# elodin-sys/elodin

Hardware: AMD Instinct MI355X
Metric: entity-steps/s (6DOF RK4) (higher is better)
Workload: dtype f64

## Files before the change

### elodin_amd/csrc/kernels.hpp

```cpp
#pragma once
#include <hip/hip_runtime.h>
#include <stdint.h>

#pragma clang fp contract(on)

namespace sixdof {

constexpr int kMaxOps = 4;
constexpr int kMaxModelCols = 128;
constexpr int kBlock = 256;

struct DevOp {
    int32_t kind;
    int32_t aux_width;
    const void* aux;
    double p[6];
};

struct StepParams {
    void* pos;
    void* vel;
    void* accel;
    void* force;
    const void* inertia;
    uint32_t n;
    uint32_t n_ticks;
    double dt_g;
    double dt;
    uint32_t n_ops;
    uint32_t vel_independent;
    uint32_t streaming;
    uint32_t hist_ring;
    uint64_t hist_slot0;
    void* hist_pos;
    void* hist_vel;
    void* hist_accel;
    void* hist_force;
    uint64_t tick0;
    uint32_t accel_in_check;
    uint32_t reserved0;
    DevOp ops[kMaxOps];
    void* model_cols[kMaxModelCols];
    void* model_hist[kMaxModelCols];
};

enum : int { kRk4 = 0, kSemiImplicit = 1, kNone = 2 };

struct StepKernel {
    const void* fn = nullptr;
    dim3 grid;
};

StepKernel select_step(const StepParams& p, int integrator, int dtype);

hipError_t launch_step(const StepParams& p, int integrator, int dtype, hipStream_t stream);

using CustomAbiFn = unsigned (*)();
using CustomLayoutFn = unsigned (*)();
using CustomLaunchFn = int (*)(const StepParams*, int integrator, int dtype, void* stream);

constexpr int kPackWidth = 10;
constexpr int kPartialForce = 9;
constexpr int kPartialWidth = 18;

struct PairParams {
    void* pos;
    void* vel;
    void* accel;
    void* force;
    const void* inertia;
    uint32_t n;
    double dt_g, dt;
    double* pack;
    double* pack_next;
    double* partial;
    uint32_t splits;
    uint32_t partial_width;
    const uint32_t* row_start;
    const uint32_t* dst;
    uint32_t n_edges;
    uint32_t n_hubs, n_hub_chunks;
    const uint32_t* hub_rows;
    const uint32_t* hub_chunk_start;
    const uint32_t* chunk_e0;
    const uint32_t* chunk_row;
    double* chunk_partial;
    int32_t pair_kind;
    double p0, p1;
    uint32_t n_ops;
    DevOp ops[kMaxOps];
    uint32_t packed;
};
uint32_t pair_splits_for(uint32_t n);
// ... 38 lines not shown
```

### elodin_amd/csrc/sixdof_capi.cpp

```cpp
#include <dlfcn.h>
#include <hip/hip_runtime.h>

#include <algorithm>
#include <chrono>
#include <cmath>
#include <cstdio>
#include <cstdlib>
#include <cstring>
#include <iterator>
#include <map>
#include <string>
#include <unordered_map>
#include <vector>

#include "../../include/sixdof_hip.h"
#include "../../include/sixdof_apollo.h"
#include "kernels.hpp"
#include "abi_guard.hpp"
#include "aql_chain.hpp"
#include "step_plan.hpp"

using namespace sixdof;

namespace {

struct Column {
    uint64_t id = 0;
    int prim = SIXDOF_PRIM_F64;
    uint64_t width = 1;
    uint64_t n_rows = 0;
    size_t elem = 8;
    size_t bytes = 0;
    std::vector<uint64_t> ids;
    void* host = nullptr;
    void* dev = nullptr;
    std::vector<uint32_t> rows;
    uint32_t* d_rows = nullptr;
    void* compact = nullptr;
    void* live = nullptr;
    bool joined = false;
    void* snap = nullptr;
    bool host_pinned = false;
};

thread_local std::string g_create_error;

struct FoldTable {
    const uint32_t* src_rows;
    const uint32_t* row_start;
    const uint32_t* dst;
    uint32_t n_src;
    uint32_t n_lane;
};
constexpr uint32_t kFoldWaveDegree = 64;

struct FoldSlot {
    bool needs_table = false;
    bool wave_ok = false;
    uint32_t count = 1, stride = 0;
    bool set = false;
    uint32_t* d_blob = nullptr;
    FoldTable table{};
};
using SetFoldTableFn = int (*)(unsigned, const FoldTable*);

double now_ms() {
    using namespace std::chrono;
    return duration<double, std::milli>(steady_clock::now().time_since_epoch()).count();
}

uint64_t cid(const char* s) { return sixdof_component_id(s); }

constexpr uint32_t kAqlSlots = 8;

struct Replay {
    StepParams key{};
    std::map<uint32_t, hipGraphExec_t> graphs;
    bool aql_off = false;
    aql::Device* aql_dev = nullptr;
    std::string aql_why;
    std::string aql_fault;
    void* aql_args = nullptr;
    std::map<uint64_t, aql::Run> aql_runs;
    uint64_t aql_slot_key[kAqlSlots] = {};
    uint32_t aql_next_spare = 2;

    void drop() {
        for (auto& kv : graphs) hipGraphExecDestroy(kv.second);
        graphs.clear();
        aql_runs.clear();
        std::fill(std::begin(aql_slot_key), std::end(aql_slot_key), 0);
        aql_next_spare = 2;
    }
    void rekey(StepParams P) {
        P.tick0 = P.hist_slot0 = 0;
        if (std::memcmp(&P, &key, sizeof(P)) != 0) drop(), key = P;
    }
    void release() {
        drop();
        if (aql_args && aql_fault.empty()) hipFree(aql_args);
        aql::release(aql_dev);
    }
};

}

struct sixdof_handle {
    sixdof_desc desc{};
    int device = 0;
    hipStream_t stream = nullptr;
    hipEvent_t ev0 = nullptr, ev1 = nullptr;
    hipEvent_t evp0 = nullptr, evp1 = nullptr;
    bool prev_pending = false;
    hipStream_t copy_stream = nullptr;
    hipEvent_t ev_snap = nullptr, ev_copied = nullptr;
    bool copy_pending = false;
    uint64_t stream_lo = 0, stream_hi = 0;
    std::vector<void*> pinned_user;
    bool step_pending = false;
    std::vector<hipEvent_t> launch_events;
    std::map<uint64_t, Column> cols;
    std::vector<sixdof_effector_op> ops;
    std::vector<uint32_t> edge_src, edge_dst;
    std::vector<uint32_t> csr_start, csr_dst;
    uint32_t* d_csr_start = nullptr;
    uint32_t* d_csr_dst = nullptr;
    uint32_t* d_hub = nullptr;
    double* d_chunk_partial = nullptr;
    uint32_t n_hubs = 0, n_hub_chunks = 0;
    void* d_scratch = nullptr;
    size_t scratch_bytes = 0;
    std::vector<uint64_t> joined_ids;
    bool identity_join = true;
    uint64_t tick = 0;
    bool bound = false;
    bool resident = false;
    sixdof_timings last{};
    void* custom_dl = nullptr;
    CustomLaunchFn custom_launch = nullptr;
    void* pair_dl = nullptr;
    CustomPairLaunchFn pair_launch = nullptr;
    std::vector<uint64_t> custom_aux;
    std::vector<uint64_t> custom_model;
    bool custom_tick_free = false;
    int pair_only_small = -1;
// ... 97 lines not shown

uint32_t sixdof_abi_version(void) { return SIXDOF_ABI_VERSION; }


int sixdof_device_count(void) try {
    int n = 0;
    if (hipGetDeviceCount(&n) != hipSuccess) return 0;
    return n;
} SIXDOF_ABI_CATCH(&g_create_error)

const char* sixdof_last_error(const sixdof_handle* h) { return h ? h->err.c_str() : g_create_error.c_str(); }

void sixdof_destroy(sixdof_handle* h);

int sixdof_create(const sixdof_desc* d, sixdof_handle** out) try {
    if (!d || !out) {
        g_create_error = "sixdof_create: null argument";
        return SIXDOF_ERR_INVALID_ARGUMENT;
    }
    *out = nullptr;
    if (d->struct_size != sizeof(sixdof_desc)) {
        g_create_error = "sixdof_create: struct_size mismatch (ABI version skew)";
        return SIXDOF_ERR_INVALID_ARGUMENT;
    }
    if (d->integrator != SIXDOF_INTEGRATOR_RK4 && d->integrator != SIXDOF_INTEGRATOR_SEMI_IMPLICIT &&
        d->integrator != SIXDOF_INTEGRATOR_NONE) {
        g_create_error = "sixdof_create: unknown integrator";
        return SIXDOF_ERR_INVALID_ARGUMENT;
    }
    if (d->dtype != SIXDOF_F64 && d->dtype != SIXDOF_F32) {
        g_create_error = "sixdof_create: unknown dtype";
        return SIXDOF_ERR_INVALID_ARGUMENT;
    }
    if (d->n_entities > 0xFFFFFFF0ull) {
        g_create_error = "sixdof_create: n_entities exceeds u32 row index range";
        return SIXDOF_ERR_INVALID_ARGUMENT;
    }
    int n_dev = 0;
    hipError_t e = hipGetDeviceCount(&n_dev);
    if (e != hipSuccess || n_dev == 0) {
        g_create_error = std::string("sixdof_create: no HIP device (") + hipGetErrorString(e) +
                         "); this backend has no CPU fallback";
        return SIXDOF_ERR_NO_DEVICE;
    }
    if (d->device_ordinal < 0 || d->device_ordinal >= n_dev) {
        g_create_error = "sixdof_create: device_ordinal out of range";
        return SIXDOF_ERR_INVALID_ARGUMENT;
    }
    auto* h = new sixdof_handle();
    h->desc = *d;
    if (h->desc.ticks_per_launch == 0) h->desc.ticks_per_launch = 1;
    const char* aql_env = std::getenv("SIXDOF_AQL");
    h->replay.aql_off = aql_env && aql_env[0] == '0';
    h->device = d->device_ordinal;
    h->id_pos = cid("world_pos");
    h->id_vel = cid("world_vel");
    h->id_accel = cid("world_accel");
    h->id_force = cid("force");
    h->id_inertia = cid("inertia");
    h->id_tick = cid("tick");
    h->id_dt = cid("simulation_time_step");
    if ((e = hipSetDevice(h->device)) != hipSuccess || (e = hipStreamCreate(&h->stream)) != hipSuccess ||
        (e = hipEventCreate(&h->ev0)) != hipSuccess || (e = hipEventCreate(&h->ev1)) != hipSuccess ||
        (e = hipEventCreate(&h->evp0)) != hipSuccess || (e = hipEventCreate(&h->evp1)) != hipSuccess) {
        g_create_error = std::string("sixdof_create: ") + hipGetErrorString(e);
        sixdof_destroy(h);
        return SIXDOF_ERR_BACKEND;
    }
    *out = h;
    return SIXDOF_OK;
} SIXDOF_ABI_CATCH(&g_create_error)

void sixdof_destroy(sixdof_handle* h) try {
    if (!h) return;
    hipSetDevice(h->device);
    if (h->stream) hipStreamSynchronize(h->stream);
    h->replay.release();
    if (h->copy_stream) hipStreamSynchronize(h->copy_stream);
    for (auto& kv : h->cols) {
        h->free_join(kv.second);
        if (kv.second.dev) hipFree(kv.second.dev);
        if (kv.second.snap) hipFree(kv.second.snap);
        if (kv.second.host_pinned) hipHostUnregister(kv.second.host);
    }
    for (void* p : h->pinned_user) (void)hipHostUnregister(p);
    if (h->copy_stream) hipStreamDestroy(h->copy_stream);
    if (h->ev_snap) hipEventDestroy(h->ev_snap);
    if (h->ev_copied) hipEventDestroy(h->ev_copied);
    if (h->d_csr_start) hipFree(h->d_csr_start);
    if (h->d_csr_dst) hipFree(h->d_csr_dst);
    if (h->d_hub) hipFree(h->d_hub);
    if (h->d_chunk_partial) hipFree(h->d_chunk_partial);
    if (h->d_scratch) hipFree(h->d_scratch);
    if (h->d_tick_refs) hipFree(h->d_tick_refs);
    h->free_fold_tables();
    for (void* p : h->d_hist) if (p) hipFree(p);
    for (void* p : h->d_model_hist) if (p) hipFree(p);
    if (h->custom_dl) dlclose(h->custom_dl);
    if (h->pair_dl) dlclose(h->pair_dl);
    for (hipEvent_t e : h->launch_events) hipEventDestroy(e);
    if (h->ev0) hipEventDestroy(h->ev0);
    if (h->ev1) hipEventDestroy(h->ev1);
    if (h->evp0) hipEventDestroy(h->evp0);
    if (h->evp1) hipEventDestroy(h->evp1);
    if (h->stream) hipStreamDestroy(h->stream);
    delete h;
// ... 950 lines not shown
        const size_t slot0 = static_cast<size_t>((first_tick - 1) % h->hist_ring);
        const size_t head = std::min<size_t>(n_ticks, h->hist_ring - slot0);
        char* dst = static_cast<char*>(host_dst[k]);
        const char* ring = static_cast<const char*>(h->d_hist[k]);
        HIP_TRY(h, hipMemcpyAsync(dst, ring + slot0 * block, head * block, hipMemcpyDeviceToHost, h->copy_stream));
        if (head < n_ticks)
            HIP_TRY(h, hipMemcpyAsync(dst + head * block, ring, (n_ticks - head) * block, hipMemcpyDeviceToHost, h->copy_stream));
    }
    HIP_TRY(h, hipEventRecord(h->ev_copied, h->copy_stream));
    h->copy_pending = true;
    h->stream_lo = first_tick;
    h->stream_hi = last;
    return SIXDOF_OK;
} SIXDOF_ABI_CATCH(err_of(h))

int sixdof_download_column(sixdof_handle* h, uint64_t component_id) try {
    if (!h) return SIXDOF_ERR_INVALID_ARGUMENT;
    Column* c = h->col(component_id);
    if (!c) return h->fail(SIXDOF_ERR_COMPONENT_NOT_FOUND, "download_column: unknown component");
    HIP_TRY(h, hipSetDevice(h->device));
    int rc = scatter_back(h, c);
    if (rc != SIXDOF_OK) return rc;
    if (c->bytes) HIP_TRY(h, hipMemcpyAsync(c->host, c->dev, c->bytes, hipMemcpyDeviceToHost, h->stream));
    HIP_TRY(h, hipStreamSynchronize(h->stream));
    return SIXDOF_OK;
} SIXDOF_ABI_CATCH(err_of(h))

int sixdof_upload_column(sixdof_handle* h, uint64_t component_id) try {
    if (!h) return SIXDOF_ERR_INVALID_ARGUMENT;
    Column* c = h->col(component_id);
    if (!c) return h->fail(SIXDOF_ERR_COMPONENT_NOT_FOUND, "upload_column: unknown component");
    if (!h->resident) return h->fail(SIXDOF_ERR_INVALID_ARGUMENT, "upload_column: nothing is resident yet (sixdof_upload first)");
    HIP_TRY(h, hipSetDevice(h->device));
    if (c->bytes) HIP_TRY(h, hipMemcpyAsync(c->dev, c->host, c->bytes, hipMemcpyHostToDevice, h->stream));
    if (c->joined && c->compact) {
        hipError_t e = launch_gather_rows(c->compact, c->dev, c->d_rows, static_cast<uint32_t>(h->joined_ids.size()),
                                          static_cast<uint32_t>(c->width), c->elem, h->stream);
        if (e != hipSuccess) return h->hip_fail(e, "gather_rows");
    }
    HIP_TRY(h, hipStreamSynchronize(h->stream));
    if (component_id == h->id_accel) h->accel_is_host_data = true;
    return SIXDOF_OK;
} SIXDOF_ABI_CATCH(err_of(h))

bool graph_eligible(const sixdof_handle* h) {
    return (h->desc.flags & SIXDOF_FLAG_USE_GRAPH) && !(h->desc.flags & SIXDOF_FLAG_TIME_EACH_LAUNCH) && !h->hist_ring &&
           (h->custom_model.empty() || h->custom_tick_free) && h->model == 0 && !h->has_pair_op();
}

static bool opens_with_check(const sixdof_handle* h, uint64_t n_ticks) {
    return h->accel_is_host_data && h->desc.integrator == SIXDOF_INTEGRATOR_RK4 && n_ticks > 0;
}

constexpr size_t kGraphCacheMax = 8;

int ensure_graph(sixdof_handle* h, const StepParams& P, uint32_t len, hipGraphExec_t* out) {
    std::map<uint32_t, hipGraphExec_t>& graphs = h->replay.graphs;
    if (auto it = graphs.find(len); it != graphs.end()) {
        *out = it->second;
        return SIXDOF_OK;
    }
    if (graphs.size() >= kGraphCacheMax) {
        for (auto g = graphs.begin(); g != graphs.end();) {
            if (g->first == kGraphLen || g->first == kGraphLong) { ++g; continue; }
            hipGraphExecDestroy(g->second);
            g = graphs.erase(g);
        }
    }
    hipGraph_t g = nullptr;
    HIP_TRY(h, hipStreamBeginCapture(h->stream, hipStreamCaptureModeThreadLocal));
    hipError_t le = hipSuccess;
    for (uint32_t i = 0; i < len && le == hipSuccess; i++) le = launch_any(h, P);
    hipError_t ce = hipStreamEndCapture(h->stream, &g);
    if (le != hipSuccess) return h->hip_fail(le, "launch_step (capture)");
    if (ce != hipSuccess) return h->hip_fail(ce, "hipStreamEndCapture");
    hipGraphExec_t exec = nullptr;
    hipError_t ie = hipGraphInstantiate(&exec, g, nullptr, nullptr, 0);
    hipGraphDestroy(g);
    if (ie != hipSuccess) return h->hip_fail(ie, "hipGraphInstantiate");
    (void)hipGraphUpload(exec, h->stream);
    graphs[len] = exec;
    *out = exec;
    return SIXDOF_OK;
}

static int ensure_plan_graphs(sixdof_handle* h, const StepParams& P, const ChainPlan& c, hipGraphExec_t g[3]) {
    int rc = SIXDOF_OK;
    if (c.open || c.n_short) rc = ensure_graph(h, P, kGraphLen, &g[0]);
    if (rc == SIXDOF_OK && c.n_long) rc = ensure_graph(h, P, kGraphLong, &g[1]);
    if (rc == SIXDOF_OK && c.tail) rc = ensure_graph(h, P, c.tail, &g[2]);
    return rc;
}


constexpr size_t kAqlSlotBytes = (sizeof(StepParams) + 255) / 256 * 256;
constexpr double kAqlStallS = 60.0;

static bool aql_run(sixdof_handle* h, const StepParams& P, uint32_t check, uint32_t ticks, aql::Run* out) {
    Replay& rp = h->replay;
    const uint64_t key = uint64_t(check) << 32 | ticks;
    if (auto it = rp.aql_runs.find(key); it != rp.aql_runs.end()) return *out = it->second, true;
    uint32_t slot_index = check;
    if (ticks != h->desc.ticks_per_launch) {
        slot_index = rp.aql_next_spare;
        rp.aql_next_spare = slot_index + 1 == kAqlSlots ? 2 : slot_index + 1;
        rp.aql_runs.erase(rp.aql_slot_key[slot_index]);
        rp.aql_slot_key[slot_index] = 0;
    }
    StepParams Q = P;
    Q.accel_in_check = check;
    Q.n_ticks = ticks;
    Q.tick0 = Q.hist_slot0 = 0;
    const StepKernel k = select_step(Q, h->desc.integrator, h->desc.dtype);
    if (!k.fn) return rp.aql_why = "no built-in kernel for this launch", false;
    aql::Run r;
    if (!aql::kernel_code(rp.aql_dev, k.fn, sizeof(StepParams), &r.code, &rp.aql_why)) return false;
    if (r.code.kernarg_align > 256) return rp.aql_why = "kernarg alignment above 256 bytes", false;
    char* slot = static_cast<char*>(rp.aql_args) + slot_index * kAqlSlotBytes;
    hipError_t e = hipMemcpy(slot, &Q, sizeof(Q), hipMemcpyHostToDevice);
    if (e != hipSuccess) return rp.aql_why = std::string("hipMemcpy (argument block): ") + hipGetErrorString(e), false;
    r.kernarg = slot;
    r.blocks = k.grid.x;
    rp.aql_runs[key] = r;
    if (slot_index >= 2) rp.aql_slot_key[slot_index] = key;
    return *out = r, true;
}

static bool aql_batch(sixdof_handle* h, const StepParams& P, const BatchPlan& b, aql::Run runs[3]) {
    const uint32_t K = h->desc.ticks_per_launch;
    if ((b.check_ticks && !aql_run(h, P, 1, b.check_ticks, &runs[0])) || (b.full && !aql_run(h, P, 0, K, &runs[1])) ||
        (b.rem && !aql_run(h, P, 0, b.rem, &runs[2])))
        return false;
    runs[0].count = b.check_ticks ? 1 : 0;
    runs[1].count = b.full;
    runs[2].count = b.rem ? 1 : 0;
    return true;
}

enum class Path { kApollo, kPair, kAql, kRigid };

struct Route {
    Path path;
    const char* why = nullptr;
    int rc = SIXDOF_OK;
    BatchPlan plan{};
};

static Route choose_path(sixdof_handle* h, uint64_t n_ticks, StepParams* P, aql::Run runs[3]) {
    if (h->model == 1) return {Path::kApollo};
    if (h->has_pair_op()) return {Path::kPair};
    Replay& rp = h->replay;
    const bool replay = graph_eligible(h);
    const char* why = nullptr;
    if (rp.aql_off) why = "SIXDOF_AQL=0";
    else if (!replay) why = "not graph-eligible";
    else if (h->custom_launch) why = "generated pipe";
    else if (h->desc.flags & SIXDOF_FLAG_ASYNC_STEP) why = "ASYNC_STEP";
    else if (h->desc.n_entities == 0) why = "no rows";
    else if (!rp.aql_why.empty()) why = rp.aql_why.c_str();
    else if (!rp.aql_fault.empty()) return {Path::kAql};
    else if (!h->resident) why = "columns not uploaded yet";
    if (!h->bound) return {Path::kRigid, why, SIXDOF_ERR_COMPONENT_NOT_FOUND};
    if (int rc = fill_step_params(h, P); rc != SIXDOF_OK) return {Path::kRigid, why ? why : h->err.c_str(), rc};
    const uint32_t K = h->desc.ticks_per_launch;
    P->n_ticks = K;
    if (replay) rp.rekey(*P);
    const BatchPlan plan = plan_batch(n_ticks, K, opens_with_check(h, n_ticks), replay);
    if (!why && !rp.aql_dev && (rp.aql_dev = aql::acquire(h->device, &rp.aql_why))) {
        if (hipError_t e = hipMalloc(&rp.aql_args, kAqlSlots * kAqlSlotBytes); e != hipSuccess)
            rp.aql_args = nullptr, rp.aql_why = std::string("hipMalloc: ") + hipGetErrorString(e);
    }
    if (!why && (!rp.aql_why.empty() || !aql_batch(h, *P, plan, runs))) why = rp.aql_why.c_str();
    return {why ? Path::kRigid : Path::kAql, why, SIXDOF_OK, plan};
}

static int prepare_batch(sixdof_handle* h, const Route& r, const StepParams& P, uint64_t n_ticks) {
    if (r.path == Path::kAql && !h->replay.aql_fault.empty()) return SIXDOF_OK;
    aql::Run runs[3];
    hipGraphExec_t unused[3] = {};
    for (bool check : {false, opens_with_check(h, n_ticks)}) {
        const BatchPlan b = plan_batch(n_ticks, h->desc.ticks_per_launch, check, true);
        if (r.path == Path::kAql) (void)aql_batch(h, P, b, runs);
        else if (int rc = ensure_plan_graphs(h, P, b.chains, unused); rc != SIXDOF_OK) return rc;
    }
    if (r.path != Path::kAql) HIP_TRY(h, hipStreamSynchronize(h->stream));
    return SIXDOF_OK;
}

int prepare_graph(sixdof_handle* h) {
    if (!h->bound || !graph_eligible(h)) return SIXDOF_OK;
    StepParams P;
    aql::Run runs[3];
    const Route r = choose_path(h, h->desc.ticks_per_launch, &P, runs);
    if (r.rc != SIXDOF_OK) return SIXDOF_OK;
    if (r.path == Path::kAql) return prepare_batch(h, r, P, h->desc.ticks_per_launch);
    hipGraphExec_t unused = nullptr;
    int rc = ensure_graph(h, P, kGraphLen, &unused);
    if (rc == SIXDOF_OK) (void)hipStreamSynchronize(h->stream);
    return rc;
}

int sixdof_prepare_step(sixdof_handle* h, uint64_t n_ticks) try {
    if (!h) return SIXDOF_ERR_INVALID_ARGUMENT;
    if (!h->bound || !h->resident) return h->fail(SIXDOF_ERR_COMPONENT_NOT_FOUND, "prepare_step: upload the columns first");
    if (!graph_eligible(h)) return SIXDOF_OK;
    HIP_TRY(h, hipSetDevice(h->device));
    StepParams P;
    aql::Run runs[3];
    const Route r = choose_path(h, n_ticks, &P, runs);
    return r.rc != SIXDOF_OK ? r.rc : prepare_batch(h, r, P, n_ticks);
} SIXDOF_ABI_CATCH(err_of(h))

const char* sixdof_step_path(sixdof_handle* h) try {
    if (!h) return "invalid handle";
    (void)hipSetDevice(h->device);
    StepParams P;
    aql::Run runs[3];
    const Route r = choose_path(h, h->desc.ticks_per_launch, &P, runs);
    if (r.path == Path::kApollo) h->path = "apollo";
    else if (r.path == Path::kPair) h->path = "pair";
    else if (r.path == Path::kAql) h->path = h->replay.aql_fault.empty() ? "aql" : "aql (failed: " + h->replay.aql_fault + ")";
    else h->path = std::string(graph_eligible(h) ? "hipgraph: " : "eager: ") + r.why;
    return h->path.c_str();
} SIXDOF_ABI_CATCH_VALUE(err_of(h), nullptr)

static int step_pair(sixdof_handle* h, uint64_t n_ticks, uint64_t* launches) {
    if (h->desc.dtype != SIXDOF_F64) return h->fail(SIXDOF_ERR_UNSUPPORTED, "step: pair effectors are f64 only");
    PairParams P;
    int rc = fill_pair_params(h, &P);
    if (rc != SIXDOF_OK) return rc;
    const char* no_small = std::getenv("SIXDOF_PAIR_SMALL");
    const bool custom = P.pair_kind == SIXDOF_EFF_EDGE_CUSTOM;
    bool small = P.n <= kPairSmallMax && !(no_small && no_small[0] == '0');
    if (custom) {
        if (!h->pair_launch) return h->fail(SIXDOF_ERR_BACKEND, "step: custom pair op without sixdof_set_custom_pair");
        if (h->pair_only_small >= 0) small = h->pair_only_small == 1;
        if (small && P.n > kPairSmallMax)
            return h->fail(SIXDOF_ERR_INVALID_ARGUMENT, "step: the pair object was generated for the one-launch small-graph kernel (<= " +
                           std::to_string(kPairSmallMax) + " rows) but the joined graph has " + std::to_string(P.n) + " rows");
    }
    const uint32_t K = h->hist_ring ? 1u : (small ? h->desc.ticks_per_launch : 1u << 20);
    const bool sets_packed = custom || !small;
    for (uint64_t done = 0; done < n_ticks;) {
        const uint32_t k = static_cast<uint32_t>(std::min<uint64_t>(K, n_ticks - done));
        if (custom) {
            hipError_t e = static_cast<hipError_t>(h->pair_launch(&P, h->desc.integrator, k, small ? 1 : 0, h->stream, launches));
            if (e != hipSuccess) return h->hip_fail(e, "custom pair launch");
        } else if (small) {
            hipError_t e = launch_pair_small(P, h->desc.integrator, k, h->stream, launches);
            if (e != hipSuccess) return h->hip_fail(e, "launch_pair_small");
        } else {
            hipError_t e = launch_pair_ticks(P, h->desc.integrator, k, h->stream, launches);
            if (e != hipSuccess) return h->hip_fail(e, "launch_pair_ticks");
        }
        done += k;
        if (sets_packed) P.packed = 1;
        if (int src = snapshot_tick_to_ring(h, h->tick + done); src != SIXDOF_OK) return src;
    }
    return SIXDOF_OK;
}

static int step_rigid(sixdof_handle* h, const StepParams& P, const BatchPlan& b, uint64_t n_ticks, uint64_t* launches) {
    const uint32_t K = h->desc.ticks_per_launch;
    const bool time_each = (h->desc.flags & SIXDOF_FLAG_TIME_EACH_LAUNCH) != 0;
    if (time_each) {
        const uint64_t need = 2 * b.launches();
        if (need > 8192) return h->fail(SIXDOF_ERR_INVALID_ARGUMENT, "step: TIME_EACH_LAUNCH supports <= 4096 launches per call");
        while (h->launch_events.size() < need) {
            hipEvent_t e = nullptr;
            HIP_TRY(h, hipEventCreate(&e));
            h->launch_events.push_back(e);
        }
    }
    auto eager = [&](StepParams Q, uint32_t ticks) -> int {
        Q.n_ticks = ticks;
        Q.tick0 = Q.hist_slot0 = h->tick + *launches * K;
        if (time_each) HIP_TRY(h, hipEventRecord(h->launch_events[2 * *launches], h->stream));
        hipError_t e = launch_any(h, Q);
        if (e != hipSuccess) return h->hip_fail(e, "launch_step");
        if (time_each) HIP_TRY(h, hipEventRecord(h->launch_events[2 * *launches + 1], h->stream));
        ++*launches;
        return SIXDOF_OK;
    };
    if (n_ticks > 0) h->accel_is_host_data = false;
    if (b.check_ticks) {
        StepParams P1 = P;
        P1.accel_in_check = 1;
        if (int rc = eager(P1, b.check_ticks); rc != SIXDOF_OK) return rc;
    }
    if (const ChainPlan& c = b.chains; c.launches()) {
        hipGraphExec_t g[3] = {};
        if (int rc = ensure_plan_graphs(h, P, c, g); rc != SIXDOF_OK) return rc;
        HIP_TRY(h, hipEventRecord(h->ev0, h->stream));
        const std::pair<hipGraphExec_t, uint64_t> replays[4] = {{g[0], c.open ? 1 : 0}, {g[1], c.n_long}, {g[0], c.n_short}, {g[2], c.tail ? 1 : 0}};
        for (const auto& [graph, times] : replays)
            for (uint64_t i = 0; i < times; i++) HIP_TRY(h, hipGraphLaunch(graph, h->stream));
        *launches += c.launches();
    }
    h->last.graph_launches = b.chains.launches();
    for (uint64_t i = b.chains.launches(); i < b.full; i++)
        if (int rc = eager(P, K); rc != SIXDOF_OK) return rc;
    return b.rem ? eager(P, b.rem) : SIXDOF_OK;
}

static int step_aql(sixdof_handle* h, const BatchPlan& b, const aql::Run runs[3], uint64_t n_ticks, uint64_t* launches) {
    Replay& rp = h->replay;
    if (!rp.aql_fault.empty()) return h->fail(SIXDOF_ERR_BACKEND, rp.aql_fault);
    for (hipStream_t s : {h->stream, static_cast<hipStream_t>(nullptr)}) {
        const hipError_t q = hipStreamQuery(s);
        if (q == hipErrorNotReady) HIP_TRY(h, hipStreamSynchronize(s));
        else if (q != hipSuccess) return h->hip_fail(q, "hipStreamQuery");
    }
    double device_ms = 0.0;
    if (!aql::run_chain(rp.aql_dev, runs, 3, kAqlStallS, &device_ms, &rp.aql_fault))
        return h->fail(SIXDOF_ERR_BACKEND, rp.aql_fault);
    if (n_ticks > 0) h->accel_is_host_data = false;
    *launches = b.launches();
    h->last.graph_launches = b.chains.launches();
    h->last.kernel_device_ms = device_ms;
    return SIXDOF_OK;
}

int sixdof_step(sixdof_handle* h, uint64_t n_ticks, sixdof_timings* tm) try {
    if (!h) return SIXDOF_ERR_INVALID_ARGUMENT;
    if (!h->bound) return h->fail(SIXDOF_ERR_COMPONENT_NOT_FOUND, "step: no columns bound");
    HIP_TRY(h, hipSetDevice(h->device));
    const double t0 = now_ms();
    const bool async_step = (h->desc.flags & SIXDOF_FLAG_ASYNC_STEP) != 0;
    if (h->step_pending || h->prev_pending) {
        std::swap(h->ev0, h->evp0);
        std::swap(h->ev1, h->evp1);
        std::swap(h->step_pending, h->prev_pending);
        if (h->step_pending) {
            float ms_prev = 0.f;
            HIP_TRY(h, hipEventSynchronize(h->ev1));
            if (hipEventElapsedTime(&ms_prev, h->ev0, h->ev1) == hipSuccess) h->last.kernel_device_ms = ms_prev;
            h->step_pending = false;
        }
    }
    if (h->hist_ring && h->copy_pending && h->stream_hi >= h->stream_lo && n_ticks) {
        const uint64_t ring = h->hist_ring, in_flight = h->stream_hi - h->stream_lo + 1;
        const uint64_t a = h->tick % ring, b = (h->stream_lo - 1) % ring;
        const uint64_t gap_ab = (b + ring - a) % ring, gap_ba = (a + ring - b) % ring;
        const bool overlap = n_ticks + in_flight > ring || gap_ab < std::min<uint64_t>(n_ticks, ring) || gap_ba < in_flight;
        if (overlap) HIP_TRY(h, hipStreamWaitEvent(h->stream, h->ev_copied, 0));
    }
    if (h->desc.integrator == SIXDOF_INTEGRATOR_NONE && (!h->custom_launch || h->model != 0 || h->has_pair_op()))
        return h->fail(SIXDOF_ERR_UNSUPPORTED, "step: SIXDOF_INTEGRATOR_NONE runs generated system programs only (sixdof_set_custom_pipe)");
    uint64_t launches = 0;
    StepParams P;
    aql::Run runs[3];
    const Route r = choose_path(h, n_ticks, &P, runs);
    if (r.rc != SIXDOF_OK) return r.rc;
    const bool aql = r.path == Path::kAql;
    if (!aql) HIP_TRY(h, hipEventRecord(h->ev0, h->stream));
    const int rc = aql                       ? step_aql(h, r.plan, runs, n_ticks, &launches)
                   : r.path == Path::kApollo ? step_apollo(h, n_ticks, &launches)
                   : r.path == Path::kPair   ? step_pair(h, n_ticks, &launches)
                                             : step_rigid(h, P, r.plan, n_ticks, &launches);
    if (rc != SIXDOF_OK) return rc;
    if (!aql) HIP_TRY(h, hipEventRecord(h->ev1, h->stream));
    if (!async_step && !aql) {
        const double spin_until = now_ms() + 0.25;
        hipError_t q = hipEventQuery(h->ev1);
        while (q == hipErrorNotReady && now_ms() < spin_until) q = hipEventQuery(h->ev1);
        if (q != hipSuccess) {
            (void)hipGetLastError();
            HIP_TRY(h, hipStreamSynchronize(h->stream));
        }
        float ms0 = 0.f;
        hipEventElapsedTime(&ms0, h->ev0, h->ev1);
        h->last.kernel_device_ms = ms0;
    }
    h->tick += n_ticks;
    h->step_pending = async_step;
    h->last.kernel_invoke_ms = now_ms() - t0;
    h->last.launches = launches;
    h->last.ticks = n_ticks;
    h->last.kernel_sum_ms = 0.0;
    if ((h->desc.flags & SIXDOF_FLAG_TIME_EACH_LAUNCH) && !h->has_pair_op()) {
        for (uint64_t i = 0; i < launches && 2 * i + 1 < h->launch_events.size(); i++) {
            float one = 0.f;
            if (hipEventElapsedTime(&one, h->launch_events[2 * i], h->launch_events[2 * i + 1]) == hipSuccess) h->last.kernel_sum_ms += one;
        }
    }
    if (tm) *tm = h->last;
    return SIXDOF_OK;
} SIXDOF_ABI_CATCH(err_of(h))


static thread_local sixdof_handle* g_tick_handle = nullptr;

int sixdof_tick_bind(sixdof_handle* h) try {
    g_tick_handle = h;
    return SIXDOF_OK;
} SIXDOF_ABI_CATCH(err_of(h))

static void tick_slot_ids(const sixdof_handle* h, std::vector<uint64_t>* in, std::vector<uint64_t>* out) {
    *in = {h->id_tick, h->id_force, h->id_inertia, h->id_pos, h->id_dt, h->id_vel, h->id_accel};
    for (auto& o : h->ops)
        if (o.aux_component_id) in->push_back(o.aux_component_id);
    std::map<uint64_t, int> ordered;
    for (uint64_t id : *in) ordered[id] = 1;
    out->clear();
// ... 59 lines not shown
```

### elodin_amd/csrc/step_kernel.hpp

```cpp
#pragma once
#include <type_traits>

#include "effectors.hpp"
#include "kernels.hpp"
#include "spatial.hpp"

namespace sixdof {

constexpr int kWave = 64;

typedef __attribute__((address_space(1))) const void* global_cptr;
typedef __attribute__((address_space(3))) void* lds_ptr;


constexpr int kPolPlain = 0, kPolNtStores = 1, kPolSc1Stores = 2, kPolNt = 9;
constexpr int pol_ld(int pol) { return pol / 8; }
constexpr int pol_st(int pol) { return pol % 8; }

template <int BYTES, int POL>
__device__ __forceinline__ void slab_dma_in(const char* __restrict__ g, char* l, uint32_t lane) {
    constexpr int kFull = BYTES / 1024, kRem = (BYTES % 1024) / 16;
    constexpr int kAux = pol_ld(POL) == 1 ? 2 : 0;
#pragma unroll
    for (int i = 0; i < kFull; i++)
// ... 108 lines not shown
    Quat<T> q0 = {T(0), T(0), T(0), T(1)};
    Vec3<T> p0 = {T(0), T(0), T(0)}, inv_I = {T(1), T(1), T(1)}, I_diag = {T(1), T(1), T(1)};
    Spatial<T> v0 = zero6, A_out = zero6, F_out = zero6;
    T mass = T(1), inv_m = T(1);
    if (active && !kDead) {
        const T* r = l_pos + t * 7;
        q0 = Quat<T>{r[0], r[1], r[2], r[3]};
        p0 = Vec3<T>{r[4], r[5], r[6]};
        const T* s = l_vel + t * 6;
        v0.ang = Vec3<T>{s[0], s[1], s[2]};
        v0.lin = Vec3<T>{s[3], s[4], s[5]};
        const T* m = l_c + t * 7;
        I_diag = Vec3<T>{m[0], m[1], m[2]};
        inv_I = Vec3<T>{recip(m[0]), recip(m[1]), recip(m[2])};
        mass = m[6];
        inv_m = recip(mass);
        if constexpr (INTEGRATOR == kNone || PIPE::kPreReadsAccel) {
            const T* a = g_accel + (size_t)t * 6;
            A_out = Spatial<T>{{a[0], a[1], a[2]}, {a[3], a[4], a[5]}};
        }
        if constexpr (INTEGRATOR == kNone) {
            const T* f = g_force + (size_t)t * 6;
            F_out = Spatial<T>{{f[0], f[1], f[2]}, {f[3], f[4], f[5]}};
        }
    }
    if (P.n_ticks == 0) return;
    __syncthreads();

    auto stage_pos = [&](const Quat<T>& q, const Vec3<T>& p) {
        if (active) {
            T* r = l_pos + t * 7;
            r[0] = q.i; r[1] = q.j; r[2] = q.k; r[3] = q.w; r[4] = p.x; r[5] = p.y; r[6] = p.z;
        }
    };
    auto stage6 = [&](T* l, const Spatial<T>& m) {
        if (active) {
            T* s = l + t * 6;
            s[0] = m.ang.x; s[1] = m.ang.y; s[2] = m.ang.z; s[3] = m.lin.x; s[4] = m.lin.y; s[5] = m.lin.z;
        }
    };
    auto flush7 = [&](const T* l, T* o, auto pol) {
        if (full) slab_out<ROWS * 7 * sizeof(T), decltype(pol)::value>(reinterpret_cast<const char*>(l), reinterpret_cast<char*>(o), t);
        else slab_out_tail(l, o, rows * 7, t);
    };
    auto flush6 = [&](const T* l, T* o, auto pol) {
        if (full) slab_out<ROWS * 6 * sizeof(T), decltype(pol)::value>(reinterpret_cast<const char*>(l), reinterpret_cast<char*>(o), t);
        else slab_out_tail(l, o, rows * 6, t);
    };
    constexpr std::integral_constant<int, POL> kLive{};
    constexpr std::integral_constant<int, 1> kRing{};

    const bool record = P.hist_pos != nullptr && P.hist_ring != 0;
    const bool early_ok = !PIPE::kHasModel && !record && !(P.streaming & 256u);
    const T dt_g = T(P.dt_g), dt = T(P.dt);
    Body<T> b;
    b.mass = mass;
    b.I = I_diag;
    Wrench<T> F = zero_wrench<T>();
    bool flushed = false;
#ifdef SIXDOF_TICK_OUT_OF_LINE
    auto one_tick = [&](auto early_tag, auto check_tag, uint32_t tick) __attribute__((noinline)) {
#else
    auto one_tick = [&](auto early_tag, auto check_tag, uint32_t tick) {
#endif
        constexpr bool early = decltype(early_tag)::value;
        const bool check = decltype(check_tag)::value || (PIPE::kHasModel && P.accel_in_check && tick == 0);
        if constexpr (PIPE::kHasModel) {
            PIPE::pre(P, P.tick0 + tick + 1, regs, q0, p0, v0, I_diag, mass, A_out);
            if constexpr (PIPE::kWritesInertia) {
                inv_I = Vec3<T>{recip(I_diag.x), recip(I_diag.y), recip(I_diag.z)};
                inv_m = recip(mass);
                b.mass = mass;
                b.I = I_diag;
            }
        }
        if constexpr (INTEGRATOR == kRk4) {
            const T h1 = dt_g * T(0.5), h3 = dt_g;
            Spatial<T> A, sv, sa;
            b.q = normalized(q0);
            b.p = p0;
            b.v = v0;
            if (check && active) {
                const T* a = g_accel + (size_t)t * 6;
                b.v.ang = b.v.ang + T(0) * Vec3<T>{a[0], a[1], a[2]};
                b.v.lin = b.v.lin + T(0) * Vec3<T>{a[3], a[4], a[5]};
            }
            F = zero_wrench<T>();
            PIPE::apply(P, aux, regs, b, F);
            A = calc_accel<PIPE>(b.q, F, inv_I, inv_m, T(0));
            sv = b.v;
            sa = A;
            b.q = integrate_world(q0, h1 * v0.ang);
            b.p = axpy(h1, v0.lin, p0);
            b.v = axpy(h1, A, v0);
            sv = axpy(T(2), b.v, sv);
            F = zero_wrench<T>();
            PIPE::apply(P, aux, regs, b, F);
            A = calc_accel<PIPE>(b.q, F, inv_I, inv_m, T(0));
            sa = axpy(T(2), A, sa);
            b.v = axpy(h1, A, v0);
            sv = axpy(T(2), b.v, sv);
            if (!PIPE::vel_independent(P)) {
                F = zero_wrench<T>();
                PIPE::apply(P, aux, regs, b, F);
                A = calc_accel<PIPE>(b.q, F, inv_I, inv_m, T(0));
            }
            sa = axpy(T(2), A, sa);
            T n3;
            b.q = integrate_world(q0, h3 * v0.ang, &n3);
            const T taint = accel_taint(n3);
            b.p = axpy(h3, v0.lin, p0);
            b.v = axpy(h3, A, v0);
            sv = sv + b.v;
            const T g = dt * T(1.0 / 6.0);
            const Quat<T> q_new = integrate_world(q0, g * sv.ang);
            const Vec3<T> p_new = axpy(g + taint, sv.lin, p0);
            if constexpr (early) {
                stage_pos(q_new, p_new);
                __syncthreads();
                flush7(l_pos, g_pos, kLive);
            }
            F = zero_wrench<T>();
            PIPE::apply(P, aux, regs, b, F);
            if constexpr (early) {
                stage6(l_force, world_wrench<PIPE>(b.q, F));
                __syncthreads();
                flush6(l_force, g_force, kLive);
            }
            A = calc_accel<PIPE>(b.q, F, inv_I, inv_m + taint, taint);
            if constexpr (early) {
                stage6(l_c, A);
                __syncthreads();
                flush6(l_c, g_accel, kLive);
            }
            sa = sa + A;
            v0 = axpy(g, sa, v0);
            q0 = q_new;
            p0 = p_new;
            A_out = A;
            if constexpr (early) {
                stage6(l_vel, v0);
                __syncthreads();
                flush6(l_vel, g_vel, kLive);
                flushed = true;
            }
        } else if constexpr (INTEGRATOR == kNone) {
        } else {
            T n0;
            b.q = normalized(q0, &n0);
            const T taint = accel_taint(n0);
            b.p = p0;
            b.v = v0;
            F = zero_wrench<T>();
            PIPE::apply(P, aux, regs, b, F);
            if constexpr (early) {
                stage6(l_force, world_wrench<PIPE>(b.q, F));
                __syncthreads();
                flush6(l_force, g_force, kLive);
            }
            const Spatial<T> A = calc_accel<PIPE>(b.q, F, inv_I, inv_m + taint, taint);
            if constexpr (early) {
                stage6(l_c, A);
                __syncthreads();
                flush6(l_c, g_accel, kLive);
            }
            v0 = axpy(dt, A, v0);
            if constexpr (early) {
                stage6(l_vel, v0);
                __syncthreads();
                flush6(l_vel, g_vel, kLive);
            }
            q0 = integrate_world(q0, dt * v0.ang);
            p0 = axpy(dt, v0.lin, p0);
            A_out = A;
            if constexpr (early) {
                stage_pos(q0, p0);
                __syncthreads();
                flush7(l_pos, g_pos, kLive);
                flushed = true;
            }
        }
        if constexpr (PIPE::kHasModel) PIPE::post(P, P.tick0 + tick + 1, regs, q0, p0, v0, I_diag, mass, A_out);
        if (record) {
            if constexpr (INTEGRATOR != kNone) F_out = world_wrench<PIPE>(b.q, F);
            const size_t slot = (size_t)((P.hist_slot0 + tick) % P.hist_ring);
            if constexpr (!kDead) {
                stage_pos(q0, p0);
                stage6(l_vel, v0);
                stage6(l_c, A_out);
                stage6(l_force, F_out);
                __syncthreads();
                const size_t r7 = (slot * P.n + row0) * 7, r6 = (slot * P.n + row0) * 6;
                flush7(l_pos, static_cast<T*>(P.hist_pos) + r7, kRing);
                flush6(l_vel, static_cast<T*>(P.hist_vel) + r6, kRing);
                flush6(l_c, static_cast<T*>(P.hist_accel) + r6, kRing);
                flush6(l_force, static_cast<T*>(P.hist_force) + r6, kRing);
            }
            if constexpr (PIPE::kHasModel)
                if (active) PIPE::record(P, slot, row0 + t, regs);
            __syncthreads();
        }
    };
    {
        constexpr std::false_type no{};
        constexpr std::true_type yes{};
        uint32_t tick = 0;
        if constexpr (PIPE::kHasModel) {
            for (; tick < P.n_ticks; tick++) one_tick(no, no, tick);
        } else {
            if constexpr (INTEGRATOR == kRk4 && CHECK)
                if (P.accel_in_check && P.n_ticks) one_tick(no, yes, tick++);
            for (; tick + 1 < P.n_ticks; tick++) one_tick(no, no, tick);
            if (tick < P.n_ticks) {
                if (early_ok) one_tick(yes, no, tick);
                else one_tick(no, no, tick);
            }
        }
    }
    if constexpr (PIPE::kHasModel) {
        if (active) {
            PIPE::template store<T, POL>(P, row0 + t, regs);
            if constexpr (PIPE::kWritesInertia) {
                T* gi = static_cast<T*>(const_cast<void*>(P.inertia)) + (size_t)(row0 + t) * 7;
                gi[0] = I_diag.x; gi[1] = I_diag.y; gi[2] = I_diag.z; gi[6] = mass;
            }
        }
    }
    if (flushed || kDead) return;
    if constexpr (INTEGRATOR != kNone) F_out = world_wrench<PIPE>(b.q, F);
    stage_pos(q0, p0);
    stage6(l_vel, v0);
    stage6(l_c, A_out);
    stage6(l_force, F_out);
    __syncthreads();
    flush7(l_pos, g_pos, kLive);
    flush6(l_vel, g_vel, kLive);
    flush6(l_c, g_accel, kLive);
    flush6(l_force, g_force, kLive);
}


template <class T, class PIPE, int POL>
inline StepKernel select_i(const StepParams& p, int integrator, dim3 grid) {
#ifdef SIXDOF_AB_BUILD
    if constexpr (!PIPE::kHasModel) {
        if ((p.streaming & 512u) && integrator == kRk4 && !p.accel_in_check)
            return {reinterpret_cast<const void*>(&sixdof_step_kernel<T, kRk4, PIPE, POL, false, 32>), dim3((p.n + 31) / 32)};
    }
#endif
    if (integrator == kRk4) {
        if constexpr (!PIPE::kHasModel) {
            if (p.accel_in_check)
                return {reinterpret_cast<const void*>(&sixdof_step_kernel<T, kRk4, PIPE, kPolPlain, true>), grid};
        }
        return {reinterpret_cast<const void*>(&sixdof_step_kernel<T, kRk4, PIPE, POL>), grid};
    }
    if (integrator == kNone) {
        if constexpr (PIPE::kHasModel) return {reinterpret_cast<const void*>(&sixdof_step_kernel<T, kNone, PIPE, POL>), grid};
        return {};
    }
    return {reinterpret_cast<const void*>(&sixdof_step_kernel<T, kSemiImplicit, PIPE, POL>), grid};
}

template <class T, class PIPE, bool SWEEP>
inline StepKernel select_t(const StepParams& p, int integrator, dim3 grid) {
    const uint32_t pol = p.streaming & 255u;
    switch (pol) {
    case kPolNt: return select_i<T, PIPE, kPolNt>(p, integrator, grid);
    case kPolNtStores: return select_i<T, PIPE, kPolNtStores>(p, integrator, grid);
    default: break;
    }
#ifdef SIXDOF_AB_BUILD
    if (pol == kPolSc1Stores) return select_i<T, PIPE, kPolSc1Stores>(p, integrator, grid);
    if constexpr (SWEEP) {
        switch (pol) {
        case 3: return select_i<T, PIPE, 3>(p, integrator, grid);
        case 4: return select_i<T, PIPE, 4>(p, integrator, grid);
        case 8: return select_i<T, PIPE, 8>(p, integrator, grid);
        case 10: return select_i<T, PIPE, 10>(p, integrator, grid);
        case 11: return select_i<T, PIPE, 11>(p, integrator, grid);
        case 12: return select_i<T, PIPE, 12>(p, integrator, grid);
        default: break;
        }
    }
#endif
    return select_i<T, PIPE, kPolPlain>(p, integrator, grid);
}

template <class PIPE, bool SWEEP = false>
// ... 7 lines not shown
```

Baseline: 13.26 billion.

## Skip accel and force writes on non-final launches in multi-launch batches

```diff
diff --git a/elodin_amd/csrc/kernels.hpp b/elodin_amd/csrc/kernels.hpp
--- a/elodin_amd/csrc/kernels.hpp
+++ b/elodin_amd/csrc/kernels.hpp
@@ -38,7 +38,7 @@
     void* hist_force;
     uint64_t tick0;
     uint32_t accel_in_check;
-    uint32_t reserved0;
+    uint32_t state_only;
     DevOp ops[kMaxOps];
     void* model_cols[kMaxModelCols];
     void* model_hist[kMaxModelCols];
diff --git a/elodin_amd/csrc/sixdof_capi.cpp b/elodin_amd/csrc/sixdof_capi.cpp
--- a/elodin_amd/csrc/sixdof_capi.cpp
+++ b/elodin_amd/csrc/sixdof_capi.cpp
@@ -72,10 +72,12 @@
 uint64_t cid(const char* s) { return sixdof_component_id(s); }
 
 constexpr uint32_t kAqlSlots = 8;
+constexpr uint32_t kAqlSpare0 = 3;
 
 struct Replay {
     StepParams key{};
     std::map<uint32_t, hipGraphExec_t> graphs;
+    bool state_only_off = false;
     bool aql_off = false;
     aql::Device* aql_dev = nullptr;
     std::string aql_why;
@@ -83,14 +85,14 @@
     void* aql_args = nullptr;
     std::map<uint64_t, aql::Run> aql_runs;
     uint64_t aql_slot_key[kAqlSlots] = {};
-    uint32_t aql_next_spare = 2;
+    uint32_t aql_next_spare = kAqlSpare0;
 
     void drop() {
         for (auto& kv : graphs) hipGraphExecDestroy(kv.second);
         graphs.clear();
         aql_runs.clear();
         std::fill(std::begin(aql_slot_key), std::end(aql_slot_key), 0);
-        aql_next_spare = 2;
+        aql_next_spare = kAqlSpare0;
     }
     void rekey(StepParams P) {
         P.tick0 = P.hist_slot0 = 0;
@@ -294,6 +296,8 @@
     if (h->desc.ticks_per_launch == 0) h->desc.ticks_per_launch = 1;
     const char* aql_env = std::getenv("SIXDOF_AQL");
     h->replay.aql_off = aql_env && aql_env[0] == '0';
+    const char* so_env = std::getenv("SIXDOF_STATE_ONLY");
+    h->replay.state_only_off = so_env && so_env[0] == '0';
     h->device = d->device_ordinal;
     h->id_pos = cid("world_pos");
     h->id_vel = cid("world_vel");
@@ -1350,25 +1354,37 @@
     return h->accel_is_host_data && h->desc.integrator == SIXDOF_INTEGRATOR_RK4 && n_ticks > 0;
 }
 
+static bool state_only_eligible(const sixdof_handle* h) {
+    return !h->replay.state_only_off && !h->custom_launch && !h->hist_ring && h->model == 0 && !h->has_pair_op();
+}
+
 constexpr size_t kGraphCacheMax = 8;
 
-int ensure_graph(sixdof_handle* h, const StepParams& P, uint32_t len, hipGraphExec_t* out) {
+enum class Chain : uint32_t { kAll = 0, kStateOnly = 1, kClosing = 2 };
+static uint32_t graph_key(uint32_t len, Chain v) { return len << 2 | static_cast<uint32_t>(v); }
+
+int ensure_graph(sixdof_handle* h, const StepParams& P, uint32_t len, Chain variant, hipGraphExec_t* out) {
     std::map<uint32_t, hipGraphExec_t>& graphs = h->replay.graphs;
-    if (auto it = graphs.find(len); it != graphs.end()) {
+    if (auto it = graphs.find(graph_key(len, variant)); it != graphs.end()) {
         *out = it->second;
         return SIXDOF_OK;
     }
     if (graphs.size() >= kGraphCacheMax) {
         for (auto g = graphs.begin(); g != graphs.end();) {
-            if (g->first == kGraphLen || g->first == kGraphLong) { ++g; continue; }
+            if (g->first >> 2 == kGraphLen || g->first >> 2 == kGraphLong) { ++g; continue; }
             hipGraphExecDestroy(g->second);
             g = graphs.erase(g);
         }
     }
+    StepParams Q = P;
+    Q.state_only = variant == Chain::kAll ? 0u : 1u;
     hipGraph_t g = nullptr;
     HIP_TRY(h, hipStreamBeginCapture(h->stream, hipStreamCaptureModeThreadLocal));
     hipError_t le = hipSuccess;
-    for (uint32_t i = 0; i < len && le == hipSuccess; i++) le = launch_any(h, P);
+    for (uint32_t i = 0; i < len && le == hipSuccess; i++) {
+        if (i + 1 == len && variant == Chain::kClosing) Q.state_only = 0;
+        le = launch_any(h, Q);
+    }
     hipError_t ce = hipStreamEndCapture(h->stream, &g);
     if (le != hipSuccess) return h->hip_fail(le, "launch_step (capture)");
     if (ce != hipSuccess) return h->hip_fail(ce, "hipStreamEndCapture");
@@ -1377,36 +1393,58 @@
     hipGraphDestroy(g);
     if (ie != hipSuccess) return h->hip_fail(ie, "hipGraphInstantiate");
     (void)hipGraphUpload(exec, h->stream);
-    graphs[len] = exec;
+    graphs[graph_key(len, variant)] = exec;
     *out = exec;
     return SIXDOF_OK;
 }
 
-static int ensure_plan_graphs(sixdof_handle* h, const StepParams& P, const ChainPlan& c, hipGraphExec_t g[3]) {
-    int rc = SIXDOF_OK;
-    if (c.open || c.n_short) rc = ensure_graph(h, P, kGraphLen, &g[0]);
-    if (rc == SIXDOF_OK && c.n_long) rc = ensure_graph(h, P, kGraphLong, &g[1]);
-    if (rc == SIXDOF_OK && c.tail) rc = ensure_graph(h, P, c.tail, &g[2]);
-    return rc;
+struct ChainReplay {
+    uint32_t len = 0;
+    Chain variant = Chain::kAll;
+    uint64_t times = 0;
+    hipGraphExec_t graph = nullptr;
+};
+
+static int ensure_plan_graphs(sixdof_handle* h, const StepParams& P, const BatchPlan& b, ChainReplay r[5]) {
+    const ChainPlan& c = b.chains;
+    const Chain v = state_only_eligible(h) ? Chain::kStateOnly : Chain::kAll;
+    r[0] = {kGraphLen, v, c.open ? 1u : 0u};
+    r[1] = {kGraphLong, v, c.n_long};
+    r[2] = {kGraphLen, v, c.n_short};
+    r[3] = {c.tail, v, c.tail ? 1u : 0u};
+    r[4] = {};
+    if (v == Chain::kStateOnly && c.launches() && c.launches() == b.full && !b.rem) {
+        int last = 3;
+        while (!r[last].times) last--;
+        r[last].times--;
+        r[4] = {r[last].len, Chain::kClosing, 1};
+    }
+    for (bool tail : {false, true})
+        for (int i = 0; i < 5; i++) {
+            if (!r[i].times || (r[i].len != kGraphLen && r[i].len != kGraphLong) != tail) continue;
+            if (int rc = ensure_graph(h, P, r[i].len, r[i].variant, &r[i].graph); rc != SIXDOF_OK) return rc;
+        }
+    return SIXDOF_OK;
 }
 
 
 constexpr size_t kAqlSlotBytes = (sizeof(StepParams) + 255) / 256 * 256;
 constexpr double kAqlStallS = 60.0;
 
-static bool aql_run(sixdof_handle* h, const StepParams& P, uint32_t check, uint32_t ticks, aql::Run* out) {
+static bool aql_run(sixdof_handle* h, const StepParams& P, uint32_t check, uint32_t state_only, uint32_t ticks, aql::Run* out) {
     Replay& rp = h->replay;
-    const uint64_t key = uint64_t(check) << 32 | ticks;
+    const uint64_t key = uint64_t(state_only) << 33 | uint64_t(check) << 32 | ticks;
     if (auto it = rp.aql_runs.find(key); it != rp.aql_runs.end()) return *out = it->second, true;
-    uint32_t slot_index = check;
+    uint32_t slot_index = state_only ? 2 : check;
     if (ticks != h->desc.ticks_per_launch) {
         slot_index = rp.aql_next_spare;
-        rp.aql_next_spare = slot_index + 1 == kAqlSlots ? 2 : slot_index + 1;
+        rp.aql_next_spare = slot_index + 1 == kAqlSlots ? kAqlSpare0 : slot_index + 1;
         rp.aql_runs.erase(rp.aql_slot_key[slot_index]);
         rp.aql_slot_key[slot_index] = 0;
     }
     StepParams Q = P;
     Q.accel_in_check = check;
+    Q.state_only = state_only;
     Q.n_ticks = ticks;
     Q.tick0 = Q.hist_slot0 = 0;
     const StepKernel k = select_step(Q, h->desc.integrator, h->desc.dtype);
@@ -1420,18 +1458,23 @@
     r.kernarg = slot;
     r.blocks = k.grid.x;
     rp.aql_runs[key] = r;
-    if (slot_index >= 2) rp.aql_slot_key[slot_index] = key;
+    if (slot_index >= kAqlSpare0) rp.aql_slot_key[slot_index] = key;
     return *out = r, true;
 }
 
-static bool aql_batch(sixdof_handle* h, const StepParams& P, const BatchPlan& b, aql::Run runs[3]) {
+constexpr size_t kAqlRuns = 4;
+
+static bool aql_batch(sixdof_handle* h, const StepParams& P, const BatchPlan& b, aql::Run runs[kAqlRuns]) {
     const uint32_t K = h->desc.ticks_per_launch;
-    if ((b.check_ticks && !aql_run(h, P, 1, b.check_ticks, &runs[0])) || (b.full && !aql_run(h, P, 0, K, &runs[1])) ||
-        (b.rem && !aql_run(h, P, 0, b.rem, &runs[2])))
+    const uint64_t closing = state_only_eligible(h) ? (b.full && !b.rem ? 1 : 0) : b.full;
+    const uint64_t state_only = b.full - closing;
+    if ((b.check_ticks && !aql_run(h, P, 1, 0, b.check_ticks, &runs[0])) || (state_only && !aql_run(h, P, 0, 1, K, &runs[1])) ||
+        (closing && !aql_run(h, P, 0, 0, K, &runs[2])) || (b.rem && !aql_run(h, P, 0, 0, b.rem, &runs[3])))
         return false;
     runs[0].count = b.check_ticks ? 1 : 0;
-    runs[1].count = b.full;
-    runs[2].count = b.rem ? 1 : 0;
+    runs[1].count = state_only;
+    runs[2].count = closing;
+    runs[3].count = b.rem ? 1 : 0;
     return true;
 }
 
@@ -1444,7 +1487,7 @@
     BatchPlan plan{};
 };
 
-static Route choose_path(sixdof_handle* h, uint64_t n_ticks, StepParams* P, aql::Run runs[3]) {
+static Route choose_path(sixdof_handle* h, uint64_t n_ticks, StepParams* P, aql::Run runs[kAqlRuns]) {
     if (h->model == 1) return {Path::kApollo};
     if (h->has_pair_op()) return {Path::kPair};
     Replay& rp = h->replay;
@@ -1474,12 +1517,12 @@
 
 static int prepare_batch(sixdof_handle* h, const Route& r, const StepParams& P, uint64_t n_ticks) {
     if (r.path == Path::kAql && !h->replay.aql_fault.empty()) return SIXDOF_OK;
-    aql::Run runs[3];
-    hipGraphExec_t unused[3] = {};
+    aql::Run runs[kAqlRuns];
+    ChainReplay unused[5];
     for (bool check : {false, opens_with_check(h, n_ticks)}) {
         const BatchPlan b = plan_batch(n_ticks, h->desc.ticks_per_launch, check, true);
         if (r.path == Path::kAql) (void)aql_batch(h, P, b, runs);
-        else if (int rc = ensure_plan_graphs(h, P, b.chains, unused); rc != SIXDOF_OK) return rc;
+        else if (int rc = ensure_plan_graphs(h, P, b, unused); rc != SIXDOF_OK) return rc;
     }
     if (r.path != Path::kAql) HIP_TRY(h, hipStreamSynchronize(h->stream));
     return SIXDOF_OK;
@@ -1488,12 +1531,12 @@
 int prepare_graph(sixdof_handle* h) {
     if (!h->bound || !graph_eligible(h)) return SIXDOF_OK;
     StepParams P;
-    aql::Run runs[3];
+    aql::Run runs[kAqlRuns];
     const Route r = choose_path(h, h->desc.ticks_per_launch, &P, runs);
     if (r.rc != SIXDOF_OK) return SIXDOF_OK;
-    if (r.path == Path::kAql) return prepare_batch(h, r, P, h->desc.ticks_per_launch);
+    if (r.path == Path::kAql) return prepare_batch(h, r, P, 2 * uint64_t(h->desc.ticks_per_launch));
     hipGraphExec_t unused = nullptr;
-    int rc = ensure_graph(h, P, kGraphLen, &unused);
+    int rc = ensure_graph(h, P, kGraphLen, state_only_eligible(h) ? Chain::kStateOnly : Chain::kAll, &unused);
     if (rc == SIXDOF_OK) (void)hipStreamSynchronize(h->stream);
     return rc;
 }
@@ -1504,7 +1547,7 @@
     if (!graph_eligible(h)) return SIXDOF_OK;
     HIP_TRY(h, hipSetDevice(h->device));
     StepParams P;
-    aql::Run runs[3];
+    aql::Run runs[kAqlRuns];
     const Route r = choose_path(h, n_ticks, &P, runs);
     return r.rc != SIXDOF_OK ? r.rc : prepare_batch(h, r, P, n_ticks);
 } SIXDOF_ABI_CATCH(err_of(h))
@@ -1513,7 +1556,7 @@
     if (!h) return "invalid handle";
     (void)hipSetDevice(h->device);
     StepParams P;
-    aql::Run runs[3];
+    aql::Run runs[kAqlRuns];
     const Route r = choose_path(h, h->desc.ticks_per_launch, &P, runs);
     if (r.path == Path::kApollo) h->path = "apollo";
     else if (r.path == Path::kPair) h->path = "pair";
@@ -1570,8 +1613,10 @@
             h->launch_events.push_back(e);
         }
     }
+    const bool may_skip = state_only_eligible(h);
     auto eager = [&](StepParams Q, uint32_t ticks) -> int {
         Q.n_ticks = ticks;
+        Q.state_only = may_skip && !Q.accel_in_check && *launches + 1 < b.launches();
         Q.tick0 = Q.hist_slot0 = h->tick + *launches * K;
         if (time_each) HIP_TRY(h, hipEventRecord(h->launch_events[2 * *launches], h->stream));
         hipError_t e = launch_any(h, Q);
@@ -1587,12 +1632,11 @@
         if (int rc = eager(P1, b.check_ticks); rc != SIXDOF_OK) return rc;
     }
     if (const ChainPlan& c = b.chains; c.launches()) {
-        hipGraphExec_t g[3] = {};
-        if (int rc = ensure_plan_graphs(h, P, c, g); rc != SIXDOF_OK) return rc;
+        ChainReplay replays[5];
+        if (int rc = ensure_plan_graphs(h, P, b, replays); rc != SIXDOF_OK) return rc;
         HIP_TRY(h, hipEventRecord(h->ev0, h->stream));
-        const std::pair<hipGraphExec_t, uint64_t> replays[4] = {{g[0], c.open ? 1 : 0}, {g[1], c.n_long}, {g[0], c.n_short}, {g[2], c.tail ? 1 : 0}};
-        for (const auto& [graph, times] : replays)
-            for (uint64_t i = 0; i < times; i++) HIP_TRY(h, hipGraphLaunch(graph, h->stream));
+        for (const ChainReplay& r : replays)
+            for (uint64_t i = 0; i < r.times; i++) HIP_TRY(h, hipGraphLaunch(r.graph, h->stream));
         *launches += c.launches();
     }
     h->last.graph_launches = b.chains.launches();
@@ -1601,7 +1645,7 @@
     return b.rem ? eager(P, b.rem) : SIXDOF_OK;
 }
 
-static int step_aql(sixdof_handle* h, const BatchPlan& b, const aql::Run runs[3], uint64_t n_ticks, uint64_t* launches) {
+static int step_aql(sixdof_handle* h, const BatchPlan& b, const aql::Run runs[kAqlRuns], uint64_t n_ticks, uint64_t* launches) {
     Replay& rp = h->replay;
     if (!rp.aql_fault.empty()) return h->fail(SIXDOF_ERR_BACKEND, rp.aql_fault);
     for (hipStream_t s : {h->stream, static_cast<hipStream_t>(nullptr)}) {
@@ -1610,7 +1654,7 @@
         else if (q != hipSuccess) return h->hip_fail(q, "hipStreamQuery");
     }
     double device_ms = 0.0;
-    if (!aql::run_chain(rp.aql_dev, runs, 3, kAqlStallS, &device_ms, &rp.aql_fault))
+    if (!aql::run_chain(rp.aql_dev, runs, kAqlRuns, kAqlStallS, &device_ms, &rp.aql_fault))
         return h->fail(SIXDOF_ERR_BACKEND, rp.aql_fault);
     if (n_ticks > 0) h->accel_is_host_data = false;
     *launches = b.launches();
@@ -1647,7 +1691,7 @@
         return h->fail(SIXDOF_ERR_UNSUPPORTED, "step: SIXDOF_INTEGRATOR_NONE runs generated system programs only (sixdof_set_custom_pipe)");
     uint64_t launches = 0;
     StepParams P;
-    aql::Run runs[3];
+    aql::Run runs[kAqlRuns];
     const Route r = choose_path(h, n_ticks, &P, runs);
     if (r.rc != SIXDOF_OK) return r.rc;
     const bool aql = r.path == Path::kAql;
diff --git a/elodin_amd/csrc/step_kernel.hpp b/elodin_amd/csrc/step_kernel.hpp
--- a/elodin_amd/csrc/step_kernel.hpp
+++ b/elodin_amd/csrc/step_kernel.hpp
@@ -184,6 +184,7 @@
 
     const bool record = P.hist_pos != nullptr && P.hist_ring != 0;
     const bool early_ok = !PIPE::kHasModel && !record && !(P.streaming & 256u);
+    const bool state_only = !PIPE::kHasModel && P.state_only != 0;
     const T dt_g = T(P.dt_g), dt = T(P.dt);
     Body<T> b;
     b.mass = mass;
@@ -255,15 +256,19 @@
             F = zero_wrench<T>();
             PIPE::apply(P, aux, regs, b, F);
             if constexpr (early) {
-                stage6(l_force, world_wrench<PIPE>(b.q, F));
-                __syncthreads();
-                flush6(l_force, g_force, kLive);
+                if (!state_only) {
+                    stage6(l_force, world_wrench<PIPE>(b.q, F));
+                    __syncthreads();
+                    flush6(l_force, g_force, kLive);
+                }
             }
             A = calc_accel<PIPE>(b.q, F, inv_I, inv_m + taint, taint);
             if constexpr (early) {
-                stage6(l_c, A);
-                __syncthreads();
-                flush6(l_c, g_accel, kLive);
+                if (!state_only) {
+                    stage6(l_c, A);
+                    __syncthreads();
+                    flush6(l_c, g_accel, kLive);
+                }
             }
             sa = sa + A;
             v0 = axpy(g, sa, v0);
@@ -286,15 +291,19 @@
             F = zero_wrench<T>();
             PIPE::apply(P, aux, regs, b, F);
             if constexpr (early) {
-                stage6(l_force, world_wrench<PIPE>(b.q, F));
-                __syncthreads();
-                flush6(l_force, g_force, kLive);
+                if (!state_only) {
+                    stage6(l_force, world_wrench<PIPE>(b.q, F));
+                    __syncthreads();
+                    flush6(l_force, g_force, kLive);
+                }
             }
             const Spatial<T> A = calc_accel<PIPE>(b.q, F, inv_I, inv_m + taint, taint);
             if constexpr (early) {
-                stage6(l_c, A);
-                __syncthreads();
-                flush6(l_c, g_accel, kLive);
+                if (!state_only) {
+                    stage6(l_c, A);
+                    __syncthreads();
+                    flush6(l_c, g_accel, kLive);
+                }
             }
             v0 = axpy(dt, A, v0);
             if constexpr (early) {
@@ -359,14 +368,17 @@
         }
     }
     if (flushed || kDead) return;
-    if constexpr (INTEGRATOR != kNone) F_out = world_wrench<PIPE>(b.q, F);
     stage_pos(q0, p0);
     stage6(l_vel, v0);
-    stage6(l_c, A_out);
-    stage6(l_force, F_out);
+    if (!state_only) {
+        if constexpr (INTEGRATOR != kNone) F_out = world_wrench<PIPE>(b.q, F);
+        stage6(l_c, A_out);
+        stage6(l_force, F_out);
+    }
     __syncthreads();
     flush7(l_pos, g_pos, kLive);
     flush6(l_vel, g_vel, kLive);
+    if (state_only) return;
     flush6(l_c, g_accel, kLive);
     flush6(l_force, g_force, kLive);
 }
```

Result: faster. 15.30 billion (median of 6 runs) (+15.4%).
